# dmlc/xgboost

Hardware: AMD Instinct MI355X
Metric: boosting_rounds_per_sec (higher is better)
Workload: dtype fp32; 1 GPU; model=higgs-1m-hist, rows_per_gpu=1000000, n_features=28, max_depth=8, max_bin=256, objective=binary:logistic, parallelism=dp1, device=cuda

## Files before the change

### xgboost_amd/backend/gpu.py

```python
from __future__ import annotations

from typing import List, Optional, Sequence, Tuple

import numpy as np
import torch

from .. import collective
from ..data import QuantizedMatrix
from ..params import TrainParam
from ..splits import SplitEntry
from .cpu import GradQuantizer

LDS_MAX_GROUP_BINS = 8192
TARGET_HIST_TASKS = 2048
MIN_ROWS_PER_TASK = 1024


def _chunk_tasks(segments: Sequence[Tuple[int, int]],
                 slots: Optional[Sequence[int]] = None,
                 target_tasks: int = TARGET_HIST_TASKS,
                 min_rows: int = MIN_ROWS_PER_TASK) -> np.ndarray:
    total = sum(e - s for s, e in segments)
    rows_per_task = max(min_rows,
                        (total + target_tasks - 1) // max(target_tasks, 1))
# ... 507 lines not shown
                "pos": torch.zeros(n_rows, dtype=torch.int32, device=dev),
                "counters": torch.empty(max(4, 1 << param.max_depth),
                                        dtype=torch.int32, device=dev),
                "hist_tasks_cap": 16384 + max_build + 8,
                "hist_tasks": torch.empty((16384 + max_build + 8, 4),
                                          dtype=torch.int32, device=dev),
                "tg_scratch": torch.empty(3 * max_build + 8,
                                          dtype=torch.int32, device=dev),
                "qg_stage": torch.empty((n_rows, 2), dtype=torch.int32,
                                        device=dev),
                "rs_stage": torch.empty(2, dtype=torch.int64, device=dev),
                "ma_stage": torch.empty(2, dtype=torch.float32,
                                        device=dev),
                "fm_stage": torch.empty(self.qm.n_features,
                                        dtype=torch.uint8, device=dev),
                "driver": self.lib.gbt_driver_create(),
            }
            pool = 2 * max_build
            if pool <= 2048:
                rec = 1 + param.max_depth * pool
                mp = n_rows // 1024 + pool + 2
                wt_bytes = (48 * rec + 8 * rec + 8 * (param.max_depth + 2)
                            + 96 * pool + 32 * pool + 16 * mp
                            + param.max_depth * pool + 32 * 1024)
                ws["wt_max_ptasks"] = mp
                ws["wt_ws"] = torch.empty(wt_bytes, dtype=torch.uint8,
                                          device=dev)
            else:
                ws["wt_max_ptasks"] = 0
                ws["wt_ws"] = None
            self._native_ws = ws
        cap = 1 << (param.max_depth + 1)
        host = {name: np.zeros(cap, dt) for name, dt in [
            ("left", np.int32), ("right", np.int32), ("parent", np.int32),
            ("split_index", np.int32), ("split_cond", np.float32),
            ("default_left", np.uint8), ("loss_chg", np.float64),
            ("sum_hess", np.float32), ("base_weight", np.float32)]}
        fmask_ptr = None
        if feature_mask is not None:
            fm = np.ascontiguousarray(feature_mask, np.uint8)
            ws["fm_stage"].copy_(
                torch.from_numpy(fm), non_blocking=True)
            fmask_ptr = self.hip.ptr(ws["fm_stage"])
        mono_dev = mono_host = None
        if monotone is not None:
            m8 = np.ascontiguousarray(monotone, np.int8)
            key = m8.tobytes()
# ... 568 lines not shown
```

### xgboost_amd/ops/__init__.py

```python
from __future__ import annotations

import ctypes
import os
from typing import Optional

import torch

_HERE = os.path.dirname(os.path.abspath(__file__))
_LIB_PATH = os.path.join(_HERE, "libgbt_hip.so")
_lib: Optional[ctypes.CDLL] = None

_c = ctypes
_p = _c.c_void_p
_i = _c.c_int
_i64 = _c.c_int64
_f = _c.c_float
_d = _c.c_double

_SIGS = {
    "gbt_hist": [_p, _p, _i, _p, _p, _p, _i, _p, _i, _p, _p, _i, _i, _p, _i, _p, _p],
    "gbt_partition": [_p, _p, _i, _p, _p, _i64, _p, _p, _p, _i, _p, _p, _p,
                      _p, _p, _p, _p, _p],
    "gbt_evaluate": [_p, _i, _i, _i, _p, _p, _p, _d, _d, _d, _d, _d, _d,
                     _p, _p, _p, _p, _p, _p, _p, _p, _p, _i, _p],
# ... 1 lines not shown
    "gbt_predict": [_p, _i64, _i, _f, _i, _p, _p, _p, _p, _p, _p, _p, _p,
                    _p, _p, _i, _i, _p, _p, _p],
    "gbt_predict_q": [_p, _i, _i64, _i, _f, _i, _p, _p, _p, _p, _p, _p, _p,
                      _p, _i, _i, _p, _p, _p],
    "gbt_leaf_partition": [_p, _p, _i, _p, _p, _p],
    "gbt_leaf_decide": [_p, _p, _i, _p, _p, _i64, _p, _p, _i, _p, _p, _p,
                        _p, _p, _p, _p],
    "gbt_copy_ranges": [_p, _p, _p, _i, _p],
    "gbt_select_best": [_p, _p, _p, _p, _i, _i, _p, _p, _p],
    "gbt_mt_evaluate": [_p, _i, _i, _i, _i, _p, _p, _p, _p,
                        _d, _d, _d, _d, _p, _p, _p, _p, _p],
    "gbt_gpair_fused": [_i, _p, _p, _p, _f, _i64, _p, _p, _p],
    "gbt_quantize": [_p, _i64, _d, _d, _p, _p, _p, _p],
    "gbt_margin_add": [_p, _p, _p, _i64, _i, _i, _p],
    "gbt_hist_cpu": [_p, _p, _i, _p, _p, _p, _p, _i, _p, _p, _i],
    "gbt_partition_cpu": [_p, _p, _i, _p, _i64, _i64, _i, _i, _i, _p, _i,
                          _i, _p],
    "gbt_evaluate_cpu": [_p, _i, _i, _i, _p, _p, _d, _d, _d, _d, _d, _d,
                         _p, _p, _p, _p],
    "gbt_hist_csr": [_p, _p, _p, _p, _p, _i, _p, _i, _p],
    "gbt_partition_csr": [_p, _p, _p, _p, _p, _i, _p, _p, _p, _p, _p, _p],
    "gbt_driver_create": [],
    "gbt_driver_destroy": [_p],
    "gbt_grow_tree": [
        _p,
        _p, _p, _i,
        _p, _p,
        _i64, _p,
        _p, _p, _p, _p,
        _p, _p, _i, _i, _i, _i,
        _p, _p, _p, _p,
        _p, _p, _p, _p, _p, _p,
        _i,
        _p, _p, _i, _p,
        _p, _i64, _i,
        _p,
        _p, _p,
        _d, _d,
        _d, _d, _d, _d, _d, _d,
        _i,
        _p, _p,
        _p,
        _p,
        _p, _p, _p, _p, _p, _p, _p, _p, _p,
        _p,
    ],
# ... 14 lines not shown
    global _lib
    if _lib is not None:
        return _lib
    if not os.path.exists(_LIB_PATH):
        try:
            from .build_ext import build
            build()
        except Exception as e:
            raise RuntimeError(
                f"HIP kernel library missing and build failed: {e}. "
                f"Run `python {os.path.join(_HERE, 'build_ext.py')}`."
            ) from e
    _lib = ctypes.CDLL(_LIB_PATH)
    for name, argtypes in _SIGS.items():
        try:
            fn = getattr(_lib, name)
        except AttributeError:
            continue
        fn.argtypes = argtypes
        fn.restype = None
    if hasattr(_lib, "gbt_driver_create"):
        _lib.gbt_driver_create.restype = _p
        _lib.gbt_grow_tree.restype = _c.c_int
    if hasattr(_lib, "gbt_partition_cpu"):
        _lib.gbt_partition_cpu.restype = _c.c_longlong
    return _lib


ALLREDUCE_FN = _c.CFUNCTYPE(None, _c.POINTER(_c.c_longlong), _c.c_longlong)


def available() -> bool:
    try:
        load()
        return True
    except RuntimeError:
        return False


def ptr(t: Optional[torch.Tensor]):
    if t is None:
        return None
    assert t.is_contiguous(), "kernel arg tensors must be contiguous"
    return _c.c_void_p(t.data_ptr())


# ... 3 lines not shown
```

### xgboost_amd/ops/cpp/driver.hip

```cpp
#include "gbt_kernels.h"

#include <hip/hip_runtime.h>

#include <algorithm>
#include <cmath>
#include <cstdio>
#include <cstdlib>
#include <cstring>
#include <vector>

namespace {

#define HIP_CHECK(x)                                    \
  do {                                                  \
    hipError_t err__ = (x);                             \
    if (err__ != hipSuccess) return -(int)err__;        \
  } while (0)

struct PinnedRing {
  static constexpr int kSlots = 6;
  void* host[kSlots] = {};
  void* dev[kSlots] = {};
  size_t cap[kSlots] = {};
  int cur = 0;
// ... 4 lines not shown
    while (want < bytes) want <<= 1;
    if (host[slot]) hipHostFree(host[slot]);
    if (dev[slot]) hipFree(dev[slot]);
    HIP_CHECK(hipHostMalloc(&host[slot], want));
    HIP_CHECK(hipMalloc(&dev[slot], want));
    cap[slot] = want;
    return 0;
  }
  int next() {
    int s = cur;
    cur = (cur + 1) % kSlots;
    return s;
  }
};

struct DriverCtx {
  PinnedRing ring;
  void* readback_host = nullptr;
  size_t readback_cap = 0;

  hipGraphExec_t wt_graph = nullptr;
  std::vector<unsigned long long> wt_key;
  std::vector<unsigned long long> wt_seen_key;
  void* wtc_host = nullptr;
  void* wtc_dev = nullptr;
  size_t wtc_cap = 0;
  hipStream_t gstream = nullptr;
  hipEvent_t gevent = nullptr;

  int ensure_gstream() {
    if (gstream == nullptr)
      HIP_CHECK(hipStreamCreateWithFlags(&gstream, hipStreamNonBlocking));
    if (gevent == nullptr)
      HIP_CHECK(hipEventCreateWithFlags(&gevent, hipEventDisableTiming));
    return 0;
  }

  int ensure_readback(size_t bytes) {
    if (readback_cap >= bytes) return 0;
    size_t want = 4096;
    while (want < bytes) want <<= 1;
    if (readback_host) hipHostFree(readback_host);
    HIP_CHECK(hipHostMalloc(&readback_host, want));
    readback_cap = want;
    return 0;
  }
  int ensure_const(size_t bytes) {
    if (wtc_cap >= bytes) return 0;
    size_t want = 4096;
    while (want < bytes) want <<= 1;
    if (wtc_host) hipHostFree(wtc_host);
    if (wtc_dev) hipFree(wtc_dev);
    HIP_CHECK(hipHostMalloc(&wtc_host, want));
    HIP_CHECK(hipMalloc(&wtc_dev, want));
    wtc_cap = want;
    return 0;
  }
  ~DriverCtx() {
    for (int i = 0; i < PinnedRing::kSlots; ++i) {
      if (ring.host[i]) hipHostFree(ring.host[i]);
      if (ring.dev[i]) hipFree(ring.dev[i]);
    }
    if (readback_host) hipHostFree(readback_host);
    if (wt_graph) (void)hipGraphExecDestroy(wt_graph);
    if (wtc_host) hipHostFree(wtc_host);
    if (wtc_dev) hipFree(wtc_dev);
    if (gstream) (void)hipStreamDestroy(gstream);
    if (gevent) (void)hipEventDestroy(gevent);
  }
};

bool WtGraphEnabled() {
  static int v = [] {
    const char* e = getenv("GBT_WT_GRAPH");
    return e ? atoi(e) : 1;
  }();
  return v != 0;
}

bool WtGraphDebug() {
  static int v = [] {
    const char* e = getenv("GBT_WT_GRAPH_DEBUG");
    return e ? atoi(e) : 0;
  }();
  return v != 0;
}

struct Node {
  int nid;
// ... 45 lines not shown
  for (auto* n : nodes) total += n->seg_end - n->seg_begin;
  long long rows_per_task =
      std::max<long long>(min_rows, (total + target_tasks - 1) / target_tasks);
  for (size_t i = 0; i < nodes.size(); ++i) {
    int b = nodes[i]->seg_begin;
    while (b < nodes[i]->seg_end) {
      int e = (int)std::min<long long>(b + rows_per_task, nodes[i]->seg_end);
      out->push_back(BlockTask{(int)i, b, e, 0});
      b = e;
    }
  }
  if (out->empty()) out->push_back(BlockTask{0, 0, 0, 0});
}

__global__ void ZeroI64Kernel(int64_t* p, long long n) {
  long long i = (long long)blockIdx.x * blockDim.x + threadIdx.x;
  long long stride = (long long)gridDim.x * blockDim.x;
  for (; i < n; i += stride) p[i] = 0;
}

__global__ void IotaKernel(int32_t* r, long long n) {
  long long i = (long long)blockIdx.x * blockDim.x + threadIdx.x;
  for (; i < n; i += (long long)gridDim.x * blockDim.x) r[i] = (int)i;
}

__global__ void SubtractHistKernel(const int64_t* __restrict__ parents,
                                   const int64_t* __restrict__ built,
                                   int64_t* __restrict__ out,
                                   const int32_t* __restrict__ parent_slot,
                                   int n_bins2, int k,
                                   int64_t* __restrict__ ps,
                                   const int64_t* __restrict__ parent_ps,
                                   const int32_t* __restrict__ kp_dev) {
  if (kp_dev != nullptr) {
    k = *kp_dev;
    out += (long long)k * n_bins2;
  }
  const long long idx = (long long)blockIdx.x * blockDim.x + threadIdx.x;
  if (ps != nullptr && idx < k) {
    ps[2 * (k + idx)] = parent_ps[2 * idx] - ps[2 * idx];
    ps[2 * (k + idx) + 1] = parent_ps[2 * idx + 1] - ps[2 * idx + 1];
  }
  const long long total = (long long)k * n_bins2;
  for (long long i = idx; i < total; i += (long long)gridDim.x * blockDim.x) {
    const int row = (int)(i / n_bins2);
    const int col = (int)(i % n_bins2);
// ... 247 lines not shown
      const int mid = (lo + hi + 1) >> 1;
      if (s_pref[mid] <= t) lo = mid; else hi = mid - 1;
    }
    const int j = lo;
    const long long idx = t - s_pref[j];
    const int b = s_b[j] + (int)(idx * rpt);
    const int e = (int)std::min<long long>((long long)b + rpt,
                                           (long long)s_e[j]);
    out_tasks[t] = BlockTask{j, b, e, 0};
  }
}

struct LeafSeg {
  int nid, begin, end;
  int parity;
};

}

extern "C" {

void* gbt_driver_create() { return new DriverCtx(); }
void gbt_driver_destroy(void* ctx) { delete (DriverCtx*)ctx; }

typedef void (*AllreduceFn)(long long* dev_ptr, long long n_elems);

int gbt_grow_tree(
    void* vctx, const uint8_t* gidx8, const uint16_t* gidx16, int n_features,
    const uint8_t* gidx8_col, const uint16_t* gidx16_col,
    long long n_rows, const int32_t* qgpair, const int32_t* cut_ptrs_dev,
    const float* cut_values_host, const int32_t* cut_ptrs_host,
    const int32_t* n_bins_feat_dev, const int32_t* feat_group_start_dev,
    const int32_t* bin_group_start_dev, int n_groups, int max_group_bins,
    int use_shared, int n_bins,
    int32_t* ridx, int32_t* ridx_out, int64_t* hist_pool_a,
    int64_t* hist_pool_b, double* eval_gain, int32_t* eval_bin,
    uint8_t* eval_dir, int64_t* eval_lsum, int64_t* eval_best,
    int32_t* pos_out, int max_nodes_level,
    int32_t* part_counters,
    BlockTask* hist_tasks_dev,
    int hist_tasks_cap,
    int32_t* tg_scratch,
    void* wt_ws,
    long long wt_ws_bytes, int wt_max_ptasks,
    const int64_t* root_sums_dev,
    const float* maxabs_dev,
// ... 28 lines not shown
  }
  int32_t* cur_ridx = ridx;
  int32_t* alt_ridx = ridx_out;

  int n_tree_nodes = 1;
  out_left[0] = -1;
  out_right[0] = -1;
  out_parent[0] = -1;

  Node root{};
  root.nid = 0;
  root.seg_begin = 0;
  root.seg_end = (int)n_rows;
  root.hist_slot = 0;
  root.lo = -INFINITY;
  root.hi = INFINITY;

  static long long hist_tasks = [] {
    const char* e = getenv("GBT_HIST_TASKS");
    long long v = e ? atoll(e) : 256;
    return v >= 64 && v <= 16384 ? v : 256;
  }();
  const long long hist_min_rows = 2048;

  if (!whole_tree) {
    std::vector<Node*> nodes{&root};
    std::vector<BlockTask> tasks;
    ChunkTasks(nodes, &tasks, hist_min_rows, hist_tasks);
    const int slot = ctx->ring.next();
    size_t bytes = tasks.size() * sizeof(BlockTask);
    if (int e = ctx->ring.ensure(slot, bytes)) return e;
    memcpy(ctx->ring.host[slot], tasks.data(), bytes);
    HIP_CHECK(hipMemcpyAsync(ctx->ring.dev[slot], ctx->ring.host[slot], bytes,
                             hipMemcpyHostToDevice, stream));
    HIP_CHECK(hipMemsetAsync(hist_pool_a, 0, hist_row * sizeof(int64_t),
                             stream));
    gbt_hist(gidx8, gidx16, n_features, qgpair, ridx,
             (const BlockTask*)ctx->ring.dev[slot], (int)tasks.size(),
             hist_pool_a, n_bins, feat_group_start_dev, bin_group_start_dev,
             n_groups, max_group_bins, cut_ptrs_dev, use_shared, nullptr,
             stream);
    if (allreduce) allreduce((long long*)hist_pool_a, hist_row);
  }

  auto evaluate_enqueue = [&](int k, std::vector<Node*>* nodes,
                              const int64_t* hists, const int64_t* ps_dev,
// ... 81 lines not shown
    *best_out = (const int64_t*)(h + off_best);
    *cnt_out = (const int32_t*)(h + off_cnt);
    return 0;
  };

  std::vector<Node> level_nodes;
  std::vector<Node> next_level;
  std::vector<LeafSeg> leaves;
  int64_t* cur_pool = hist_pool_a;
  int64_t* next_pool = hist_pool_b;

  if (whole_tree) {
    const int choice_global = (allreduce != nullptr || has_mono) ? 1 : 0;
    const int pool = 2 * max_nodes_level;
    const int rec_slots = 1 + max_depth * pool;
    size_t off = 0;
    auto carve = [&](size_t bytes) {
      size_t o = off;
      off = (off + bytes + 255) & ~255ULL;
      return o;
    };
    const size_t o_best = carve((size_t)rec_slots * 6 * 8);
    const size_t o_seg = carve((size_t)rec_slots * 2 * 4);
    const size_t o_kn = carve((size_t)(max_depth + 2) * 4);
    const size_t o_kp = carve((size_t)(max_depth + 2) * 4);
    const size_t o_descw = carve((size_t)pool * 16);
    const size_t o_featw = carve((size_t)pool * 4);
    const size_t o_sbinw = carve((size_t)pool * 4);
    const size_t o_dlw = carve((size_t)pool);
    const size_t o_cntw = carve((size_t)pool * 8);
    const size_t o_pt = carve((size_t)wt_max_ptasks * sizeof(BlockTask));
    const size_t o_pps = carve((size_t)pool * 16);
    const size_t o_pslot = carve((size_t)pool * 4);
    const size_t o_psa = carve((size_t)pool * 16);
    const size_t o_psb = carve((size_t)pool * 16);
    const size_t o_bnda = has_mono ? carve((size_t)pool * 16) : 0;
    const size_t o_bndb = has_mono ? carve((size_t)pool * 16) : 0;
    const size_t o_mode = carve((size_t)max_depth * pool);
    if ((long long)off > wt_ws_bytes) return -9997;
    char* w = (char*)wt_ws;
    int64_t* best_rec = (int64_t*)(w + o_best);
    int32_t* seg_rec = (int32_t*)(w + o_seg);
    int32_t* kn_arr = (int32_t*)(w + o_kn);
    int32_t* kp_arr = (int32_t*)(w + o_kp);
    int32_t* d_desc = (int32_t*)(w + o_descw);
    int32_t* d_feat = (int32_t*)(w + o_featw);
    int32_t* d_sbin = (int32_t*)(w + o_sbinw);
    uint8_t* d_dl = (uint8_t*)(w + o_dlw);
    int32_t* d_cnt = (int32_t*)(w + o_cntw);
    BlockTask* d_pt = (BlockTask*)(w + o_pt);
    int64_t* d_pps = (int64_t*)(w + o_pps);
    int32_t* d_pslot = (int32_t*)(w + o_pslot);
    int64_t* ps_bufs[2] = {(int64_t*)(w + o_psa), (int64_t*)(w + o_psb)};
    double* bnd_bufs[2] = {
        has_mono ? (double*)(w + o_bnda) : nullptr,
        has_mono ? (double*)(w + o_bndb) : nullptr};
    uint8_t* d_mode = (uint8_t*)(w + o_mode);

    std::vector<BlockTask> rtasks;
    {
      std::vector<Node*> rnodes{&root};
      ChunkTasks(rnodes, &rtasks, hist_min_rows, hist_tasks);
    }
    const size_t c_tasks_off = 16;
    if (int e = ctx->ensure_const(c_tasks_off +
                                  rtasks.size() * sizeof(BlockTask)))
      return e;
    {
      int32_t* hh = (int32_t*)ctx->wtc_host;
      hh[0] = 1;
      hh[1] = 0;
      hh[2] = 0;
      hh[3] = (int)n_rows;
      memcpy((char*)ctx->wtc_host + c_tasks_off, rtasks.data(),
             rtasks.size() * sizeof(BlockTask));
    }
    const int wt_max_htasks = (int)std::min<long long>(
        std::min<long long>(n_rows / hist_min_rows, hist_tasks) +
            max_nodes_level + 1,
        (long long)hist_tasks_cap);
    size_t r_best = 0;
    size_t r_seg = ((size_t)rec_slots * 48 + 63) & ~63ULL;
    size_t r_kp = (r_seg + (size_t)rec_slots * 8 + 63) & ~63ULL;
    size_t r_rs = (r_kp + (size_t)(max_depth + 2) * 4 + 63) & ~63ULL;
    size_t r_ma = r_rs + 16;
    size_t r_mode = (r_ma + 8 + 63) & ~63ULL;
    size_t r_total = r_mode + (size_t)max_depth * pool;
    if (int e = ctx->ensure_readback(r_total)) return e;
    char* rb = (char*)ctx->readback_host;

    auto stage_h2d = [&](hipStream_t cs) -> int {
      char* ch = (char*)ctx->wtc_host;
      HIP_CHECK(hipMemcpyAsync(kn_arr, ch, 4, hipMemcpyHostToDevice,
                               cs));
      HIP_CHECK(hipMemcpyAsync(kp_arr, ch + 4, 4, hipMemcpyHostToDevice,
                               cs));
      HIP_CHECK(hipMemcpyAsync(seg_rec, ch + 8, 8, hipMemcpyHostToDevice,
                               cs));
      HIP_CHECK(hipMemcpyAsync((char*)ctx->wtc_dev + c_tasks_off,
                               ch + c_tasks_off,
                               rtasks.size() * sizeof(BlockTask),
                               hipMemcpyHostToDevice, cs));
      return 0;
    };
    auto enqueue_chain = [&](hipStream_t cs) -> int {
      int32_t* cr = ridx;
      int32_t* ar = ridx_out;
      int64_t* cp = hist_pool_a;
      int64_t* np2 = hist_pool_b;
      {
        int blocks = (int)std::min<long long>((n_rows + 255) / 256, 4096);
        hipLaunchKernelGGL(IotaKernel, dim3(blocks), dim3(256), 0, cs,
                           cr, n_rows);
      }
      {
        int zb = (int)std::min<long long>((hist_row + 255) / 256, 4096);
        hipLaunchKernelGGL(ZeroI64Kernel, dim3(zb), dim3(256), 0, cs, cp,
                           hist_row);
      }
      gbt_hist(gidx8, gidx16, n_features, qgpair, cr,
               (const BlockTask*)((char*)ctx->wtc_dev + c_tasks_off),
               (int)rtasks.size(), cp, n_bins, feat_group_start_dev,
               bin_group_start_dev, n_groups, max_group_bins, cut_ptrs_dev,
               use_shared, nullptr, cs);
      if (allreduce) allreduce((long long*)cp, hist_row);
      gbt_evaluate_masked(cp, 1, n_bins, n_features, cut_ptrs_dev,
                   root_sums_dev, maxabs_dev, 0.0, 0.0, reg_lambda,
                   reg_alpha, max_delta_step, min_child_weight,
                   has_mono ? monotone_dev : nullptr, nullptr,
                   0 , fmask_dev,
                   nullptr, eval_gain, eval_bin, eval_dir, eval_lsum,
                   nullptr, 0, cs);
      gbt_select_best(eval_gain, eval_bin, eval_dir, eval_lsum, 1,
                      n_features, best_rec, nullptr, cs);
      const int64_t* ps_prev = root_sums_dev;
      for (int L = 0; L + 1 < max_depth; ++L) {
        const int64_t* bl =
            best_rec + (L == 0 ? 0 : (1 + (size_t)(L - 1) * pool) * 6);
        const int32_t* sl =
            seg_rec + (L == 0 ? 0 : (1 + (size_t)(L - 1) * pool) * 2);
        int64_t* bo = best_rec + (1 + (size_t)L * pool) * 6;
        int32_t* so = seg_rec + (1 + (size_t)L * pool) * 2;
        int64_t* ps_next = ps_bufs[L & 1];
        const int cap_kids =
            (int)std::min<long long>(2LL << L, (long long)pool);
        hipLaunchKernelGGL(ApplyKernel, dim3(1), dim3(256), 0, cs, bl,
                           sl, kn_arr + L, kp_arr + L, ps_prev, gamma,
                           cut_ptrs_dev,
                           (long long)1024, (long long)2048, wt_max_ptasks,
                           kn_arr + L + 1, kp_arr + L + 1, d_feat, d_sbin,
                           d_dl, d_cnt, d_pt, d_desc, d_pps, d_pslot,
                           choice_global, maxabs_dev,
                           has_mono ? monotone_dev : nullptr,
                           reg_lambda, reg_alpha, max_delta_step,
                           (L == 0 || !has_mono) ? nullptr
                                                 : bnd_bufs[(L - 1) & 1],
                           has_mono ? bnd_bufs[L & 1] : nullptr,
                           L == 0 ? nullptr : d_mode + (size_t)(L - 1) * pool);
        gbt_partition(gidx8, gidx16, n_features, gidx8_col, gidx16_col,
                      n_rows, cr, ar, d_pt,
                      wt_max_ptasks, d_feat, d_sbin, d_dl, nullptr, nullptr,
                      n_bins_feat_dev, d_cnt, cs);
        std::swap(cr, ar);
        hipLaunchKernelGGL(HistTaskGenKernel, dim3(1), dim3(256), 0, cs,
                           d_cnt, d_desc, 0, hist_min_rows, hist_tasks,
                           wt_max_htasks, tg_scratch, hist_tasks_dev,
                           ps_next, kp_arr + L + 1, so,
                           allreduce != nullptr ? 2 * cap_kids : 0,
                           d_mode + (size_t)L * pool);
        {
          const long long zn = (long long)cap_kids * hist_row;
          int zb = (int)std::min<long long>((zn + 255) / 256, 4096);
          hipLaunchKernelGGL(ZeroI64Kernel, dim3(zb), dim3(256), 0, cs,
                             np2, zn);
        }
        gbt_hist(gidx8, gidx16, n_features, qgpair, cr, hist_tasks_dev,
                 wt_max_htasks, np2, n_bins, feat_group_start_dev,
                 bin_group_start_dev, n_groups, max_group_bins,
                 cut_ptrs_dev, use_shared, ps_next, cs);
        if (allreduce) {
          allreduce((long long*)np2,
                    (long long)(cap_kids / 2) * hist_row);
          allreduce((long long*)ps_next, (long long)cap_kids);
        }
// ... 1 lines not shown
          const long long total = (long long)(cap_kids / 2 + 1) * hist_row;
          int blocks = (int)std::min<long long>((total + 255) / 256, 4096);
          hipLaunchKernelGGL(SubtractHistKernel, dim3(blocks), dim3(256), 0,
                             cs, cp, np2, np2, d_pslot,
                             (int)hist_row, 0, ps_next, d_pps,
                             kp_arr + L + 1);
        }
        gbt_evaluate_masked(np2, cap_kids, n_bins, n_features, cut_ptrs_dev,
                     ps_next, maxabs_dev, 0.0, 0.0, reg_lambda, reg_alpha,
                     max_delta_step, min_child_weight,
                     has_mono ? monotone_dev : nullptr,
                     has_mono ? bnd_bufs[L & 1] : nullptr,
                     0 , fmask_dev, nullptr, eval_gain,
                     eval_bin, eval_dir, eval_lsum, kn_arr + L + 1, 0,
                     cs);
        gbt_select_best(eval_gain, eval_bin, eval_dir, eval_lsum, cap_kids,
                        n_features, bo, kn_arr + L + 1, cs);
        ps_prev = ps_next;
        std::swap(cp, np2);
      }
      return 0;
    };
    auto readback = [&](hipStream_t cs) -> int {
      HIP_CHECK(hipMemcpyAsync(rb + r_best, best_rec,
                               (size_t)rec_slots * 48,
                               hipMemcpyDeviceToHost, cs));
      HIP_CHECK(hipMemcpyAsync(rb + r_seg, seg_rec, (size_t)rec_slots * 8,
                               hipMemcpyDeviceToHost, cs));
      HIP_CHECK(hipMemcpyAsync(rb + r_kp, kp_arr,
                               (size_t)(max_depth + 2) * 4,
                               hipMemcpyDeviceToHost, cs));
      HIP_CHECK(hipMemcpyAsync(rb + r_rs, root_sums_dev, 16,
                               hipMemcpyDeviceToHost, cs));
      HIP_CHECK(hipMemcpyAsync(rb + r_ma, maxabs_dev, 8,
                               hipMemcpyDeviceToHost, cs));
      HIP_CHECK(hipMemcpyAsync(rb + r_mode, d_mode,
                               (size_t)max_depth * pool,
                               hipMemcpyDeviceToHost, cs));
      return 0;
    };

    bool enqueued = false;
    if (allreduce == nullptr && WtGraphEnabled() &&
        ctx->ensure_gstream() == 0) {
      auto db = [](double d) {
        unsigned long long u;
        memcpy(&u, &d, 8);
        return u;
      };
      std::vector<unsigned long long> key = {
          (unsigned long long)gidx8, (unsigned long long)gidx16,
          (unsigned long long)gidx8_col, (unsigned long long)gidx16_col,
          (unsigned long long)qgpair, (unsigned long long)cut_ptrs_dev,
          (unsigned long long)n_bins_feat_dev,
          (unsigned long long)feat_group_start_dev,
          (unsigned long long)bin_group_start_dev,
          (unsigned long long)ridx, (unsigned long long)ridx_out,
          (unsigned long long)hist_pool_a, (unsigned long long)hist_pool_b,
          (unsigned long long)eval_gain, (unsigned long long)eval_bin,
          (unsigned long long)eval_dir, (unsigned long long)eval_lsum,
          (unsigned long long)hist_tasks_dev,
          (unsigned long long)tg_scratch, (unsigned long long)wt_ws,
          (unsigned long long)root_sums_dev,
          (unsigned long long)maxabs_dev, (unsigned long long)monotone_dev,
          (unsigned long long)fmask_dev,
          (unsigned long long)ctx->readback_host,
          (unsigned long long)ctx->wtc_host,
          (unsigned long long)ctx->wtc_dev,
          (unsigned long long)n_rows, (unsigned long long)n_features,
          (unsigned long long)n_bins, (unsigned long long)use_shared,
          (unsigned long long)n_groups,
          (unsigned long long)max_group_bins,
          (unsigned long long)max_depth,
          (unsigned long long)max_nodes_level,
          (unsigned long long)wt_max_ptasks,
          (unsigned long long)hist_tasks_cap,
          (unsigned long long)rtasks.size(),
          (unsigned long long)has_mono,
          db(reg_lambda), db(reg_alpha), db(max_delta_step),
          db(min_child_weight), db(gamma)};
      HIP_CHECK(hipEventRecord(ctx->gevent, stream));
      HIP_CHECK(hipEventSynchronize(ctx->gevent));
      if (ctx->wt_graph != nullptr && key == ctx->wt_key) {
        if (int e = stage_h2d(ctx->gstream)) return e;
        if (hipGraphLaunch(ctx->wt_graph, ctx->gstream) == hipSuccess) {
          enqueued = true;
          if (WtGraphDebug()) fprintf(stderr, "[wtgraph] replay\n");
        } else {
          (void)hipGetLastError();
          (void)hipGraphExecDestroy(ctx->wt_graph);
          ctx->wt_graph = nullptr;
          ctx->wt_key.clear();
        }
      }
      if (!enqueued && key != ctx->wt_seen_key) {
        ctx->wt_seen_key = key;
      } else if (!enqueued) {
        if (int e = stage_h2d(ctx->gstream)) return e;
        if (hipStreamBeginCapture(ctx->gstream,
                                  hipStreamCaptureModeRelaxed) !=
            hipSuccess) {
          (void)hipGetLastError();
          goto graph_done;
        }
        int ec = enqueue_chain(ctx->gstream);
        hipGraph_t g = nullptr;
        hipError_t ce = hipStreamEndCapture(ctx->gstream, &g);
        if (WtGraphDebug())
          fprintf(stderr, "[wtgraph] capture ec=%d end=%d\n", ec, (int)ce);
        if (ec != 0) {
          if (g) (void)hipGraphDestroy(g);
          return ec;
        }
        if (ce == hipSuccess && g != nullptr) {
          if (ctx->wt_graph) {
            (void)hipGraphExecDestroy(ctx->wt_graph);
            ctx->wt_graph = nullptr;
          }
          ctx->wt_key.clear();
          hipError_t ie =
              hipGraphInstantiate(&ctx->wt_graph, g, nullptr, nullptr, 0);
// ... 8 lines not shown
            enqueued = true;
          } else if (ctx->wt_graph) {
            (void)hipGraphExecDestroy(ctx->wt_graph);
            ctx->wt_graph = nullptr;
          }
          (void)hipGraphDestroy(g);
        } else {
          (void)hipGetLastError();
        }
      }
    graph_done:
      if (!enqueued) {
        hipStreamCaptureStatus st = hipStreamCaptureStatusNone;
        if (hipStreamIsCapturing(ctx->gstream, &st) == hipSuccess &&
            st != hipStreamCaptureStatusNone) {
          hipGraph_t junk = nullptr;
          (void)hipStreamEndCapture(ctx->gstream, &junk);
          if (junk) (void)hipGraphDestroy(junk);
        }
      }
    }
    if (!enqueued) {
      if (WtGraphDebug()) fprintf(stderr, "[wtgraph] direct enqueue\n");
      if (int e = stage_h2d(stream)) return e;
      if (int e = enqueue_chain(stream)) return e;
      if (int e = readback(stream)) return e;
    } else {
      if (int e = readback(ctx->gstream)) return e;
      HIP_CHECK(hipStreamSynchronize(ctx->gstream));
    }
    HIP_CHECK(hipStreamSynchronize(stream));
    if ((max_depth - 1) & 1) std::swap(cur_ridx, alt_ridx);
    const int64_t* h_best = (const int64_t*)(rb + r_best);
    const int32_t* h_seg = (const int32_t*)(rb + r_seg);
    const int32_t* h_kp = (const int32_t*)(rb + r_kp);
    const int64_t* h_rs = (const int64_t*)(rb + r_rs);
    const float* h_ma = (const float*)(rb + r_ma);
    const uint8_t* h_mode = (const uint8_t*)(rb + r_mode);
    g_scale = h_ma[0] > 0.f ? 1073741824.0 / (double)h_ma[0] : 1.0;
    h_scale = h_ma[1] > 0.f ? 1073741824.0 / (double)h_ma[1] : 1.0;
    inv_g = 1.0 / g_scale;
    inv_h = 1.0 / h_scale;
    if (out_scales != nullptr) {
      out_scales[0] = g_scale;
      out_scales[1] = h_scale;
    }
    root.gq = h_rs[0];
    root.hq = h_rs[1];
    out_base_weight[0] =
        (float)CalcWeight(root.gq * inv_g, root.hq * inv_h, p);
    out_sum_hess[0] = (float)(root.hq * inv_h);
    {
      double gn;
      memcpy(&gn, &h_best[0], 8);
      root.bin = (int)h_best[1];
      root.dir = (int)h_best[2];
      root.lgq = h_best[3];
      root.lhq = h_best[4];
      root.feature = (int)h_best[5];
      root.gain = (root.bin >= 0 && std::isfinite(gn)) ? gn : -INFINITY;
    }
// ... 485 lines not shown
```

### xgboost_amd/ops/cpp/partition.hip

```cpp
#include "gbt_kernels.h"

#ifndef GBT_PART_BLOCK
#define GBT_PART_BLOCK 256
#endif

__device__ __forceinline__ bool DecideLeft(int local_bin, int fbins,
                                           int split_bin_local,
                                           bool default_left,
                                           const uint32_t* cat_bits,
                                           int cat_words) {
  if (local_bin >= fbins) {
    return default_left;
  }
  if (cat_words > 0) {
    const int w = local_bin >> 5;
    const bool in_set =
        (w < cat_words) && ((cat_bits[w] >> (local_bin & 31)) & 1u);
    return !in_set;
  }
  return local_bin <= split_bin_local;
}

template <typename BinT>
__global__ __launch_bounds__(GBT_PART_BLOCK) void PartitionKernel(
    const BinT* __restrict__ gidx, int n_features,
    const BinT* __restrict__ gidx_col, long long col_ld,
    const int32_t* __restrict__ ridx_in, int32_t* __restrict__ ridx_out,
    const BlockTask* __restrict__ tasks,
    const int32_t* __restrict__ split_feature,
    const int32_t* __restrict__ split_bin_local,
    const uint8_t* __restrict__ default_left,
    const uint32_t* __restrict__ cat_bits,
    const int32_t* __restrict__ cat_bits_offset,
    const int32_t* __restrict__ n_bins_feat,
    int32_t* __restrict__ counters) {
  const BlockTask task = tasks[blockIdx.x];
  if (task.row_begin >= task.row_end) return;
  const int slot = task.out_slot;
  const int feature = split_feature[slot];
  const int sbin = split_bin_local[slot];
  const bool dleft = default_left[slot] != 0;
  const int fbins = n_bins_feat[feature];
  const uint32_t* cats = nullptr;
  int cat_words = 0;
  if (cat_bits_offset != nullptr) {
    const int c0 = cat_bits_offset[slot];
    cat_words = cat_bits_offset[slot + 1] - c0;
    if (cat_words > 0) cats = cat_bits + c0;
  }

  const int n_rows = task.row_end - task.row_begin;
  const int chunk = (n_rows + (int)blockDim.x - 1) / (int)blockDim.x;
  const int my_begin = task.row_begin + (int)threadIdx.x * chunk;
  const int my_end = min(my_begin + chunk, task.row_end);

  constexpr int kMaxCacheRows = 65536;
  __shared__ uint32_t decide_bits[kMaxCacheRows / 32];
  const bool use_cache = n_rows <= kMaxCacheRows;
  if (use_cache) {
    const int n_words = (n_rows + 31) / 32;
    for (int i = threadIdx.x; i < n_words; i += blockDim.x) {
      decide_bits[i] = 0u;
    }
    __syncthreads();
  }

  const BinT* col = gidx_col ? gidx_col + (size_t)feature * col_ld
                             : nullptr;
  int my_left = 0;
  for (int i = my_begin; i < my_end; ++i) {
    const int row = ridx_in[i];
    const int local = col ? (int)col[row]
                          : (int)gidx[(size_t)row * n_features + feature];
    const bool left = DecideLeft(local, fbins, sbin, dleft, cats, cat_words);
    my_left += left ? 1 : 0;
    if (use_cache) {
      const int k = i - task.row_begin;
      if (left) atomicOr(&decide_bits[k >> 5], 1u << (k & 31));
    }
  }
  const int my_rows = max(my_end - my_begin, 0);
  const int my_right = my_rows - my_left;

  __shared__ int wave_left[GBT_PART_BLOCK / 64];
  __shared__ int wave_right[GBT_PART_BLOCK / 64];
  __shared__ int base_l, base_r;
  const int lane = threadIdx.x & 63;
  const int wave = threadIdx.x >> 6;
  int scan_l = my_left, scan_r = my_right;
  for (int off = 1; off < 64; off <<= 1) {
    const int tl = __shfl_up(scan_l, off, 64);
    const int tr = __shfl_up(scan_r, off, 64);
    if (lane >= off) {
      scan_l += tl;
      scan_r += tr;
    }
  }
  if (lane == 63) {
    wave_left[wave] = scan_l;
    wave_right[wave] = scan_r;
  }
  __syncthreads();
  int wl_off = 0, wr_off = 0;
  for (int w = 0; w < wave; ++w) {
    wl_off += wave_left[w];
    wr_off += wave_right[w];
  }
  const int excl_l = scan_l - my_left + wl_off;
  const int excl_r = scan_r - my_right + wr_off;
  if (threadIdx.x == (int)blockDim.x - 1) {
    const int tot_l = excl_l + my_left;
    const int tot_r = excl_r + my_right;
    base_l = tot_l ? atomicAdd(&counters[2 * slot], tot_l) : 0;
    base_r = tot_r ? atomicSub(&counters[2 * slot + 1], tot_r) - tot_r : 0;
  }
  __syncthreads();

  int dl = base_l + excl_l;
  int dr = base_r + excl_r;
  for (int i = my_begin; i < my_end; ++i) {
    const int row = ridx_in[i];
    bool left;
    if (use_cache) {
      const int k = i - task.row_begin;
      left = (decide_bits[k >> 5] >> (k & 31)) & 1u;
    } else {
      const int local = col ? (int)col[row]
                            : (int)gidx[(size_t)row * n_features + feature];
      left = DecideLeft(local, fbins, sbin, dleft, cats, cat_words);
    }
    if (left) {
      ridx_out[dl++] = row;
    } else {
      ridx_out[dr++] = row;
    }
  }
}

extern "C" void gbt_partition(
    const uint8_t* gidx8, const uint16_t* gidx16, int n_features,
    const uint8_t* gidx8_col, const uint16_t* gidx16_col, int64_t col_ld,
    const int32_t* ridx_in, int32_t* ridx_out, const BlockTask* tasks,
    int n_tasks, const int32_t* split_feature, const int32_t* split_bin_local,
    const uint8_t* default_left, const uint32_t* cat_bits,
    const int32_t* cat_bits_offset, const int32_t* n_bins_feat,
    int32_t* counters, hipStream_t stream) {
  if (gidx8 != nullptr) {
    hipLaunchKernelGGL((PartitionKernel<uint8_t>), dim3(n_tasks),
                       dim3(GBT_PART_BLOCK), 0, stream, gidx8, n_features,
                       gidx8_col, (long long)col_ld,
                       ridx_in, ridx_out, tasks, split_feature,
                       split_bin_local, default_left, cat_bits,
                       cat_bits_offset, n_bins_feat, counters);
  } else {
    hipLaunchKernelGGL((PartitionKernel<uint16_t>), dim3(n_tasks),
                       dim3(GBT_PART_BLOCK), 0, stream, gidx16, n_features,
                       gidx16_col, (long long)col_ld,
                       ridx_in, ridx_out, tasks, split_feature,
// ... 98 lines not shown
```

Baseline: 931.9 rounds/s.

## Rewrite partition kernel with wave ballots and fuse whole-tree init on device

The partition kernel now has each wave classify 64 consecutive rows with ballot and mbcnt, keeping decisions in registers instead of per-thread strided chunks with LDS atomicOr bit caches. Writes become coalesced within a wave, and there are separate tile-count variants by task size. Host-side root task staging and H2D copies are replaced by a fused device init kernel that also does iota and zeroing, and the readback is packed into one contiguous memcpy. Partition task granularity becomes tunable (default 4096 rows, launching fewer partition tasks). A debug check function for root tasks is also added.

```diff
diff --git a/xgboost_amd/backend/gpu.py b/xgboost_amd/backend/gpu.py
--- a/xgboost_amd/backend/gpu.py
+++ b/xgboost_amd/backend/gpu.py
@@ -553,7 +553,7 @@
                 mp = n_rows // 1024 + pool + 2
                 wt_bytes = (48 * rec + 8 * rec + 8 * (param.max_depth + 2)
                             + 96 * pool + 32 * pool + 16 * mp
-                            + param.max_depth * pool + 32 * 1024)
+                            + param.max_depth * pool + 24 + 32 * 1024)
                 ws["wt_max_ptasks"] = mp
                 ws["wt_ws"] = torch.empty(wt_bytes, dtype=torch.uint8,
                                           device=dev)
diff --git a/xgboost_amd/ops/__init__.py b/xgboost_amd/ops/__init__.py
--- a/xgboost_amd/ops/__init__.py
+++ b/xgboost_amd/ops/__init__.py
@@ -47,6 +47,7 @@
     "gbt_partition_csr": [_p, _p, _p, _p, _p, _i, _p, _p, _p, _p, _p, _p],
     "gbt_driver_create": [],
     "gbt_driver_destroy": [_p],
+    "gbt_root_tasks_check": [_i64, _i64, _i64, _p],
     "gbt_grow_tree": [
         _p,
         _p, _p, _i,
@@ -107,6 +108,8 @@
     if hasattr(_lib, "gbt_driver_create"):
         _lib.gbt_driver_create.restype = _p
         _lib.gbt_grow_tree.restype = _c.c_int
+    if hasattr(_lib, "gbt_root_tasks_check"):
+        _lib.gbt_root_tasks_check.restype = _c.c_int
     if hasattr(_lib, "gbt_partition_cpu"):
         _lib.gbt_partition_cpu.restype = _c.c_longlong
     return _lib
diff --git a/xgboost_amd/ops/cpp/driver.hip b/xgboost_amd/ops/cpp/driver.hip
--- a/xgboost_amd/ops/cpp/driver.hip
+++ b/xgboost_amd/ops/cpp/driver.hip
@@ -50,9 +50,6 @@
   hipGraphExec_t wt_graph = nullptr;
   std::vector<unsigned long long> wt_key;
   std::vector<unsigned long long> wt_seen_key;
-  void* wtc_host = nullptr;
-  void* wtc_dev = nullptr;
-  size_t wtc_cap = 0;
   hipStream_t gstream = nullptr;
   hipEvent_t gevent = nullptr;
 
@@ -73,17 +70,6 @@
     readback_cap = want;
     return 0;
   }
-  int ensure_const(size_t bytes) {
-    if (wtc_cap >= bytes) return 0;
-    size_t want = 4096;
-    while (want < bytes) want <<= 1;
-    if (wtc_host) hipHostFree(wtc_host);
-    if (wtc_dev) hipFree(wtc_dev);
-    HIP_CHECK(hipHostMalloc(&wtc_host, want));
-    HIP_CHECK(hipMalloc(&wtc_dev, want));
-    wtc_cap = want;
-    return 0;
-  }
   ~DriverCtx() {
     for (int i = 0; i < PinnedRing::kSlots; ++i) {
       if (ring.host[i]) hipHostFree(ring.host[i]);
@@ -91,8 +77,6 @@
     }
     if (readback_host) hipHostFree(readback_host);
     if (wt_graph) (void)hipGraphExecDestroy(wt_graph);
-    if (wtc_host) hipHostFree(wtc_host);
-    if (wtc_dev) hipFree(wtc_dev);
     if (gstream) (void)hipStreamDestroy(gstream);
     if (gevent) (void)hipEventDestroy(gevent);
   }
@@ -184,6 +168,45 @@
 __global__ void IotaKernel(int32_t* r, long long n) {
   long long i = (long long)blockIdx.x * blockDim.x + threadIdx.x;
   for (; i < n; i += (long long)gridDim.x * blockDim.x) r[i] = (int)i;
+}
+
+long long RootRowsPerTask(long long n_rows, long long min_rows,
+                          long long target_tasks) {
+  return std::max<long long>(min_rows,
+                             (n_rows + target_tasks - 1) / target_tasks);
+}
+int RootTaskCount(long long n_rows, long long rpt) {
+  return (int)std::max<long long>(1, (n_rows + rpt - 1) / rpt);
+}
+
+__global__ void WtInitKernel(int32_t* r, long long n, int64_t* zero,
+                             long long zero_n, int32_t* kn, int32_t* kp,
+                             int32_t* seg, BlockTask* root_tasks,
+                             int n_root_tasks, long long rpt,
+                             const int64_t* __restrict__ root_sums,
+                             const float* __restrict__ maxabs,
+                             int64_t* rs_out ) {
+  const long long stride = (long long)gridDim.x * blockDim.x;
+  const long long i0 = (long long)blockIdx.x * blockDim.x + threadIdx.x;
+  for (long long i = i0; i < n; i += stride) r[i] = (int)i;
+  for (long long i = i0; i < zero_n; i += stride) zero[i] = 0;
+  if (blockIdx.x != 0) return;
+  if (threadIdx.x == 0) {
+    kn[0] = 1;
+    kp[0] = 0;
+    seg[0] = 0;
+    seg[1] = (int)n;
+    rs_out[0] = root_sums[0];
+    rs_out[1] = root_sums[1];
+    float* ma = (float*)(rs_out + 2);
+    ma[0] = maxabs[0];
+    ma[1] = maxabs[1];
+  }
+  for (int t = threadIdx.x; t < n_root_tasks; t += blockDim.x) {
+    const long long b = (long long)t * rpt;
+    root_tasks[t] =
+        BlockTask{0, (int)b, (int)std::min<long long>(b + rpt, n), 0};
+  }
 }
 
 __global__ void SubtractHistKernel(const int64_t* __restrict__ parents,
@@ -477,6 +500,48 @@
 
 void* gbt_driver_create() { return new DriverCtx(); }
 void gbt_driver_destroy(void* ctx) { delete (DriverCtx*)ctx; }
+
+int gbt_root_tasks_check(long long n_rows, long long min_rows,
+                         long long target_tasks, void* stream_v) {
+  hipStream_t stream = (hipStream_t)stream_v;
+  Node root{};
+  root.seg_end = (int)n_rows;
+  std::vector<Node*> nodes{&root};
+  std::vector<BlockTask> want;
+  ChunkTasks(nodes, &want, min_rows, target_tasks);
+  const long long rpt = RootRowsPerTask(n_rows, min_rows, target_tasks);
+  const int nt = RootTaskCount(n_rows, rpt);
+  const size_t o_tasks = 192;
+  const size_t o_ridx = o_tasks + (size_t)nt * sizeof(BlockTask);
+  const size_t bytes = o_ridx + (size_t)std::max<long long>(n_rows, 1) * 4;
+  char* d = nullptr;
+  HIP_CHECK(hipMalloc((void**)&d, bytes));
+  int rc = 0;
+  std::vector<BlockTask> got(nt);
+  hipError_t e = hipMemsetAsync(d, 0, o_tasks, stream);
+  if (e == hipSuccess) {
+    int32_t* sc = (int32_t*)d;
+    hipLaunchKernelGGL(WtInitKernel, dim3(2), dim3(256), 0, stream,
+                       (int32_t*)(d + o_ridx), n_rows, (int64_t*)nullptr,
+                       0LL, sc, sc + 1, sc + 2, (BlockTask*)(d + o_tasks),
+                       nt, rpt, (const int64_t*)(d + 64),
+                       (const float*)(d + 80), (int64_t*)(d + 128));
+    e = hipMemcpyAsync(got.data(), d + o_tasks,
+                       (size_t)nt * sizeof(BlockTask), hipMemcpyDeviceToHost,
+                       stream);
+  }
+  if (e == hipSuccess) e = hipStreamSynchronize(stream);
+  (void)hipFree(d);
+  if (e != hipSuccess) return -(int)e;
+  if (want.size() != got.size()) return (int)std::max(want.size(), got.size());
+  for (size_t i = 0; i < want.size(); ++i) {
+    if (want[i].out_slot != got[i].out_slot ||
+        want[i].row_begin != got[i].row_begin ||
+        want[i].row_end != got[i].row_end)
+      ++rc;
+  }
+  return rc;
+}
 
 typedef void (*AllreduceFn)(long long* dev_ptr, long long n_elems);
 
@@ -551,6 +616,11 @@
     return v >= 64 && v <= 16384 ? v : 256;
   }();
   const long long hist_min_rows = 2048;
+  static long long part_min_rows = [] {
+    const char* e = getenv("GBT_PART_ROWS");
+    long long v = e ? atoll(e) : 4096;
+    return v >= 1024 && v <= 65536 && (v & (v - 1)) == 0 ? v : 4096;
+  }();
 
   if (!whole_tree) {
     std::vector<Node*> nodes{&root};
@@ -678,8 +748,11 @@
     };
     const size_t o_best = carve((size_t)rec_slots * 6 * 8);
     const size_t o_seg = carve((size_t)rec_slots * 2 * 4);
+    const size_t o_kp = carve((size_t)(max_depth + 2) * 4);
+    const size_t o_mode = carve((size_t)max_depth * pool);
+    const size_t o_rs = carve(24);
+    const size_t r_total = o_rs + 24;
     const size_t o_kn = carve((size_t)(max_depth + 2) * 4);
-    const size_t o_kp = carve((size_t)(max_depth + 2) * 4);
     const size_t o_descw = carve((size_t)pool * 16);
     const size_t o_featw = carve((size_t)pool * 4);
     const size_t o_sbinw = carve((size_t)pool * 4);
@@ -692,7 +765,6 @@
     const size_t o_psb = carve((size_t)pool * 16);
     const size_t o_bnda = has_mono ? carve((size_t)pool * 16) : 0;
     const size_t o_bndb = has_mono ? carve((size_t)pool * 16) : 0;
-    const size_t o_mode = carve((size_t)max_depth * pool);
     if ((long long)off > wt_ws_bytes) return -9997;
     char* w = (char*)wt_ws;
     int64_t* best_rec = (int64_t*)(w + o_best);
@@ -713,52 +785,20 @@
         has_mono ? (double*)(w + o_bndb) : nullptr};
     uint8_t* d_mode = (uint8_t*)(w + o_mode);
 
-    std::vector<BlockTask> rtasks;
-    {
-      std::vector<Node*> rnodes{&root};
-      ChunkTasks(rnodes, &rtasks, hist_min_rows, hist_tasks);
-    }
-    const size_t c_tasks_off = 16;
-    if (int e = ctx->ensure_const(c_tasks_off +
-                                  rtasks.size() * sizeof(BlockTask)))
-      return e;
-    {
-      int32_t* hh = (int32_t*)ctx->wtc_host;
-      hh[0] = 1;
-      hh[1] = 0;
-      hh[2] = 0;
-      hh[3] = (int)n_rows;
-      memcpy((char*)ctx->wtc_host + c_tasks_off, rtasks.data(),
-             rtasks.size() * sizeof(BlockTask));
-    }
+    const long long root_rpt =
+        RootRowsPerTask(n_rows, hist_min_rows, hist_tasks);
+    const int n_root_tasks = RootTaskCount(n_rows, root_rpt);
+    if (n_root_tasks > hist_tasks_cap) return -9996;
+    int64_t* d_rs = (int64_t*)(w + o_rs);
     const int wt_max_htasks = (int)std::min<long long>(
         std::min<long long>(n_rows / hist_min_rows, hist_tasks) +
             max_nodes_level + 1,
         (long long)hist_tasks_cap);
-    size_t r_best = 0;
-    size_t r_seg = ((size_t)rec_slots * 48 + 63) & ~63ULL;
-    size_t r_kp = (r_seg + (size_t)rec_slots * 8 + 63) & ~63ULL;
-    size_t r_rs = (r_kp + (size_t)(max_depth + 2) * 4 + 63) & ~63ULL;
-    size_t r_ma = r_rs + 16;
-    size_t r_mode = (r_ma + 8 + 63) & ~63ULL;
-    size_t r_total = r_mode + (size_t)max_depth * pool;
+    const int n_ptasks = (int)std::min<long long>(
+        n_rows / part_min_rows + pool + 2, (long long)wt_max_ptasks);
     if (int e = ctx->ensure_readback(r_total)) return e;
     char* rb = (char*)ctx->readback_host;
 
-    auto stage_h2d = [&](hipStream_t cs) -> int {
-      char* ch = (char*)ctx->wtc_host;
-      HIP_CHECK(hipMemcpyAsync(kn_arr, ch, 4, hipMemcpyHostToDevice,
-                               cs));
-      HIP_CHECK(hipMemcpyAsync(kp_arr, ch + 4, 4, hipMemcpyHostToDevice,
-                               cs));
-      HIP_CHECK(hipMemcpyAsync(seg_rec, ch + 8, 8, hipMemcpyHostToDevice,
-                               cs));
-      HIP_CHECK(hipMemcpyAsync((char*)ctx->wtc_dev + c_tasks_off,
-                               ch + c_tasks_off,
-                               rtasks.size() * sizeof(BlockTask),
-                               hipMemcpyHostToDevice, cs));
-      return 0;
-    };
     auto enqueue_chain = [&](hipStream_t cs) -> int {
       int32_t* cr = ridx;
       int32_t* ar = ridx_out;
@@ -766,17 +806,15 @@
       int64_t* np2 = hist_pool_b;
       {
         int blocks = (int)std::min<long long>((n_rows + 255) / 256, 4096);
-        hipLaunchKernelGGL(IotaKernel, dim3(blocks), dim3(256), 0, cs,
-                           cr, n_rows);
-      }
-      {
-        int zb = (int)std::min<long long>((hist_row + 255) / 256, 4096);
-        hipLaunchKernelGGL(ZeroI64Kernel, dim3(zb), dim3(256), 0, cs, cp,
-                           hist_row);
+        hipLaunchKernelGGL(WtInitKernel, dim3(std::max(blocks, 1)),
+                           dim3(256), 0, cs, cr, n_rows, cp, hist_row,
+                           kn_arr, kp_arr, seg_rec, hist_tasks_dev,
+                           n_root_tasks, root_rpt, root_sums_dev, maxabs_dev,
+                           d_rs);
       }
       gbt_hist(gidx8, gidx16, n_features, qgpair, cr,
-               (const BlockTask*)((char*)ctx->wtc_dev + c_tasks_off),
-               (int)rtasks.size(), cp, n_bins, feat_group_start_dev,
+               hist_tasks_dev, n_root_tasks, cp, n_bins,
+               feat_group_start_dev,
                bin_group_start_dev, n_groups, max_group_bins, cut_ptrs_dev,
                use_shared, nullptr, cs);
       if (allreduce) allreduce((long long*)cp, hist_row);
@@ -803,7 +841,7 @@
         hipLaunchKernelGGL(ApplyKernel, dim3(1), dim3(256), 0, cs, bl,
                            sl, kn_arr + L, kp_arr + L, ps_prev, gamma,
                            cut_ptrs_dev,
-                           (long long)1024, (long long)2048, wt_max_ptasks,
+                           part_min_rows, (long long)2048, n_ptasks,
                            kn_arr + L + 1, kp_arr + L + 1, d_feat, d_sbin,
                            d_dl, d_cnt, d_pt, d_desc, d_pps, d_pslot,
                            choice_global, maxabs_dev,
@@ -815,7 +853,7 @@
                            L == 0 ? nullptr : d_mode + (size_t)(L - 1) * pool);
         gbt_partition(gidx8, gidx16, n_features, gidx8_col, gidx16_col,
                       n_rows, cr, ar, d_pt,
-                      wt_max_ptasks, d_feat, d_sbin, d_dl, nullptr, nullptr,
+                      n_ptasks, d_feat, d_sbin, d_dl, nullptr, nullptr,
                       n_bins_feat_dev, d_cnt, cs);
         std::swap(cr, ar);
         hipLaunchKernelGGL(HistTaskGenKernel, dim3(1), dim3(256), 0, cs,
@@ -863,20 +901,7 @@
       return 0;
     };
     auto readback = [&](hipStream_t cs) -> int {
-      HIP_CHECK(hipMemcpyAsync(rb + r_best, best_rec,
-                               (size_t)rec_slots * 48,
-                               hipMemcpyDeviceToHost, cs));
-      HIP_CHECK(hipMemcpyAsync(rb + r_seg, seg_rec, (size_t)rec_slots * 8,
-                               hipMemcpyDeviceToHost, cs));
-      HIP_CHECK(hipMemcpyAsync(rb + r_kp, kp_arr,
-                               (size_t)(max_depth + 2) * 4,
-                               hipMemcpyDeviceToHost, cs));
-      HIP_CHECK(hipMemcpyAsync(rb + r_rs, root_sums_dev, 16,
-                               hipMemcpyDeviceToHost, cs));
-      HIP_CHECK(hipMemcpyAsync(rb + r_ma, maxabs_dev, 8,
-                               hipMemcpyDeviceToHost, cs));
-      HIP_CHECK(hipMemcpyAsync(rb + r_mode, d_mode,
-                               (size_t)max_depth * pool,
+      HIP_CHECK(hipMemcpyAsync(rb, w + o_best, r_total,
                                hipMemcpyDeviceToHost, cs));
       return 0;
     };
@@ -906,8 +931,6 @@
           (unsigned long long)maxabs_dev, (unsigned long long)monotone_dev,
           (unsigned long long)fmask_dev,
           (unsigned long long)ctx->readback_host,
-          (unsigned long long)ctx->wtc_host,
-          (unsigned long long)ctx->wtc_dev,
           (unsigned long long)n_rows, (unsigned long long)n_features,
           (unsigned long long)n_bins, (unsigned long long)use_shared,
           (unsigned long long)n_groups,
@@ -916,14 +939,17 @@
           (unsigned long long)max_nodes_level,
           (unsigned long long)wt_max_ptasks,
           (unsigned long long)hist_tasks_cap,
-          (unsigned long long)rtasks.size(),
+          (unsigned long long)n_root_tasks,
+          (unsigned long long)root_rpt,
+          (unsigned long long)part_min_rows,
+          (unsigned long long)n_ptasks,
+          (unsigned long long)wt_max_htasks,
           (unsigned long long)has_mono,
           db(reg_lambda), db(reg_alpha), db(max_delta_step),
           db(min_child_weight), db(gamma)};
       HIP_CHECK(hipEventRecord(ctx->gevent, stream));
       HIP_CHECK(hipEventSynchronize(ctx->gevent));
       if (ctx->wt_graph != nullptr && key == ctx->wt_key) {
-        if (int e = stage_h2d(ctx->gstream)) return e;
         if (hipGraphLaunch(ctx->wt_graph, ctx->gstream) == hipSuccess) {
           enqueued = true;
           if (WtGraphDebug()) fprintf(stderr, "[wtgraph] replay\n");
@@ -937,7 +963,6 @@
       if (!enqueued && key != ctx->wt_seen_key) {
         ctx->wt_seen_key = key;
       } else if (!enqueued) {
-        if (int e = stage_h2d(ctx->gstream)) return e;
         if (hipStreamBeginCapture(ctx->gstream,
                                   hipStreamCaptureModeRelaxed) !=
             hipSuccess) {
@@ -992,7 +1017,6 @@
     }
     if (!enqueued) {
       if (WtGraphDebug()) fprintf(stderr, "[wtgraph] direct enqueue\n");
-      if (int e = stage_h2d(stream)) return e;
       if (int e = enqueue_chain(stream)) return e;
       if (int e = readback(stream)) return e;
     } else {
@@ -1001,12 +1025,12 @@
     }
     HIP_CHECK(hipStreamSynchronize(stream));
     if ((max_depth - 1) & 1) std::swap(cur_ridx, alt_ridx);
-    const int64_t* h_best = (const int64_t*)(rb + r_best);
-    const int32_t* h_seg = (const int32_t*)(rb + r_seg);
-    const int32_t* h_kp = (const int32_t*)(rb + r_kp);
-    const int64_t* h_rs = (const int64_t*)(rb + r_rs);
-    const float* h_ma = (const float*)(rb + r_ma);
-    const uint8_t* h_mode = (const uint8_t*)(rb + r_mode);
+    const int64_t* h_best = (const int64_t*)(rb + o_best);
+    const int32_t* h_seg = (const int32_t*)(rb + o_seg);
+    const int32_t* h_kp = (const int32_t*)(rb + o_kp);
+    const int64_t* h_rs = (const int64_t*)(rb + o_rs);
+    const float* h_ma = (const float*)(rb + o_rs + 16);
+    const uint8_t* h_mode = (const uint8_t*)(rb + o_mode);
     g_scale = h_ma[0] > 0.f ? 1073741824.0 / (double)h_ma[0] : 1.0;
     h_scale = h_ma[1] > 0.f ? 1073741824.0 / (double)h_ma[1] : 1.0;
     inv_g = 1.0 / g_scale;
diff --git a/xgboost_amd/ops/cpp/partition.hip b/xgboost_amd/ops/cpp/partition.hip
--- a/xgboost_amd/ops/cpp/partition.hip
+++ b/xgboost_amd/ops/cpp/partition.hip
@@ -3,6 +3,13 @@
 #ifndef GBT_PART_BLOCK
 #define GBT_PART_BLOCK 256
 #endif
+
+namespace {
+constexpr int kPartWaves = GBT_PART_BLOCK / 64;
+constexpr int kPartTilesSmall = 4;
+constexpr int kPartTilesLarge = 16;
+constexpr int kPartCacheRows = kPartTilesLarge * 64 * kPartWaves;
+}
 
 __device__ __forceinline__ bool DecideLeft(int local_bin, int fbins,
                                            int split_bin_local,
@@ -19,6 +26,132 @@
     return !in_set;
   }
   return local_bin <= split_bin_local;
+}
+
+template <typename BinT>
+struct PartSplit {
+  const BinT* gidx;
+  const BinT* col;
+  int n_features, feature, fbins, sbin, cat_words;
+  bool dleft;
+  const uint32_t* cats;
+
+  __device__ __forceinline__ bool Left(int row) const {
+    const int local = col ? (int)col[row]
+                          : (int)gidx[(size_t)row * n_features + feature];
+    return DecideLeft(local, fbins, sbin, dleft, cats, cat_words);
+  }
+};
+
+__device__ __forceinline__ int LanesBelow(unsigned long long m) {
+  return (int)__builtin_amdgcn_mbcnt_hi(
+      (unsigned)(m >> 32), __builtin_amdgcn_mbcnt_lo((unsigned)m, 0u));
+}
+
+__device__ __forceinline__ void ReserveWindows(int wave_left, int wave_right,
+                                               int32_t* counters, int slot,
+                                               int* dl, int* dr) {
+  __shared__ int s_left[kPartWaves], s_right[kPartWaves];
+  __shared__ int s_base_l, s_base_r;
+  const int lane = threadIdx.x & 63;
+  const int wave = threadIdx.x >> 6;
+  if (lane == 0) {
+    s_left[wave] = wave_left;
+    s_right[wave] = wave_right;
+  }
+  __syncthreads();
+  if (threadIdx.x == 0) {
+    int tot_l = 0, tot_r = 0;
+    for (int w = 0; w < kPartWaves; ++w) {
+      tot_l += s_left[w];
+      tot_r += s_right[w];
+    }
+    s_base_l = tot_l ? atomicAdd(&counters[2 * slot], tot_l) : 0;
+    s_base_r = tot_r ? atomicSub(&counters[2 * slot + 1], tot_r) - tot_r : 0;
+  }
+  __syncthreads();
+  int l = s_base_l, r = s_base_r;
+  for (int w = 0; w < wave; ++w) {
+    l += s_left[w];
+    r += s_right[w];
+  }
+  *dl = l;
+  *dr = r;
+}
+
+template <typename BinT, int TILES>
+__device__ __forceinline__ void PartitionCached(
+    const PartSplit<BinT>& sp, const int32_t* __restrict__ ridx_in,
+    int32_t* __restrict__ ridx_out, int begin, int end, int slot,
+    int32_t* counters) {
+  const int lane = threadIdx.x & 63;
+  const int wave = threadIdx.x >> 6;
+  int rows[TILES];
+  unsigned long long lmask[TILES];
+  int wave_left = 0, wave_rows = 0;
+#pragma unroll
+  for (int j = 0; j < TILES; ++j) {
+    const int i = begin + (j * kPartWaves + wave) * 64 + lane;
+    const bool valid = i < end;
+    rows[j] = ridx_in[min(i, end - 1)];
+    lmask[j] = __ballot(sp.Left(rows[j]) && valid);
+    wave_left += __popcll(lmask[j]);
+    wave_rows += __popcll(__ballot(valid));
+  }
+  int dl, dr;
+  ReserveWindows(wave_left, wave_rows - wave_left, counters, slot, &dl, &dr);
+#pragma unroll
+  for (int j = 0; j < TILES; ++j) {
+    const int i = begin + (j * kPartWaves + wave) * 64 + lane;
+    const bool valid = i < end;
+    const unsigned long long lm = lmask[j];
+    const unsigned long long rm = __ballot(valid) & ~lm;
+    if (valid) {
+      if ((lm >> lane) & 1ull) {
+        ridx_out[dl + LanesBelow(lm)] = rows[j];
+      } else {
+        ridx_out[dr + LanesBelow(rm)] = rows[j];
+      }
+    }
+    dl += __popcll(lm);
+    dr += __popcll(rm);
+  }
+}
+
+template <typename BinT>
+__device__ __forceinline__ void PartitionRegather(
+    const PartSplit<BinT>& sp, const int32_t* __restrict__ ridx_in,
+    int32_t* __restrict__ ridx_out, int begin, int end, int slot,
+    int32_t* counters) {
+  const int lane = threadIdx.x & 63;
+  const int wave = threadIdx.x >> 6;
+  int wave_left = 0, wave_rows = 0;
+  for (int t0 = begin + wave * 64; t0 < end; t0 += kPartWaves * 64) {
+    const int i = t0 + lane;
+    const bool valid = i < end;
+    const int row = ridx_in[min(i, end - 1)];
+    wave_left += __popcll(__ballot(sp.Left(row) && valid));
+    wave_rows += __popcll(__ballot(valid));
+  }
+  int dl, dr;
+  ReserveWindows(wave_left, wave_rows - wave_left, counters, slot, &dl, &dr);
+  for (int t0 = begin + wave * 64; t0 < end; t0 += kPartWaves * 64) {
+    const int i = t0 + lane;
+    const bool valid = i < end;
+    const int row = ridx_in[min(i, end - 1)];
+    const bool left = sp.Left(row) && valid;
+    const unsigned long long lm = __ballot(left);
+    const unsigned long long rm = __ballot(valid) & ~lm;
+    if (valid) {
+      if (left) {
+        ridx_out[dl + LanesBelow(lm)] = row;
+      } else {
+        ridx_out[dr + LanesBelow(rm)] = row;
+      }
+    }
+    dl += __popcll(lm);
+    dr += __popcll(rm);
+  }
 }
 
 template <typename BinT>
@@ -37,103 +170,34 @@
   const BlockTask task = tasks[blockIdx.x];
   if (task.row_begin >= task.row_end) return;
   const int slot = task.out_slot;
-  const int feature = split_feature[slot];
-  const int sbin = split_bin_local[slot];
-  const bool dleft = default_left[slot] != 0;
-  const int fbins = n_bins_feat[feature];
-  const uint32_t* cats = nullptr;
-  int cat_words = 0;
+  PartSplit<BinT> sp;
+  sp.gidx = gidx;
+  sp.n_features = n_features;
+  sp.feature = split_feature[slot];
+  sp.sbin = split_bin_local[slot];
+  sp.dleft = default_left[slot] != 0;
+  sp.fbins = n_bins_feat[sp.feature];
+  sp.cats = nullptr;
+  sp.cat_words = 0;
   if (cat_bits_offset != nullptr) {
     const int c0 = cat_bits_offset[slot];
-    cat_words = cat_bits_offset[slot + 1] - c0;
-    if (cat_words > 0) cats = cat_bits + c0;
-  }
+    sp.cat_words = cat_bits_offset[slot + 1] - c0;
+    if (sp.cat_words > 0) sp.cats = cat_bits + c0;
+  }
+  sp.col = gidx_col ? gidx_col + (size_t)sp.feature * col_ld : nullptr;
 
   const int n_rows = task.row_end - task.row_begin;
-  const int chunk = (n_rows + (int)blockDim.x - 1) / (int)blockDim.x;
-  const int my_begin = task.row_begin + (int)threadIdx.x * chunk;
-  const int my_end = min(my_begin + chunk, task.row_end);
-
-  constexpr int kMaxCacheRows = 65536;
-  __shared__ uint32_t decide_bits[kMaxCacheRows / 32];
-  const bool use_cache = n_rows <= kMaxCacheRows;
-  if (use_cache) {
-    const int n_words = (n_rows + 31) / 32;
-    for (int i = threadIdx.x; i < n_words; i += blockDim.x) {
-      decide_bits[i] = 0u;
-    }
-    __syncthreads();
-  }
-
-  const BinT* col = gidx_col ? gidx_col + (size_t)feature * col_ld
-                             : nullptr;
-  int my_left = 0;
-  for (int i = my_begin; i < my_end; ++i) {
-    const int row = ridx_in[i];
-    const int local = col ? (int)col[row]
-                          : (int)gidx[(size_t)row * n_features + feature];
-    const bool left = DecideLeft(local, fbins, sbin, dleft, cats, cat_words);
-    my_left += left ? 1 : 0;
-    if (use_cache) {
-      const int k = i - task.row_begin;
-      if (left) atomicOr(&decide_bits[k >> 5], 1u << (k & 31));
-    }
-  }
-  const int my_rows = max(my_end - my_begin, 0);
-  const int my_right = my_rows - my_left;
-
-  __shared__ int wave_left[GBT_PART_BLOCK / 64];
-  __shared__ int wave_right[GBT_PART_BLOCK / 64];
-  __shared__ int base_l, base_r;
-  const int lane = threadIdx.x & 63;
-  const int wave = threadIdx.x >> 6;
-  int scan_l = my_left, scan_r = my_right;
-  for (int off = 1; off < 64; off <<= 1) {
-    const int tl = __shfl_up(scan_l, off, 64);
-    const int tr = __shfl_up(scan_r, off, 64);
-    if (lane >= off) {
-      scan_l += tl;
-      scan_r += tr;
-    }
-  }
-  if (lane == 63) {
-    wave_left[wave] = scan_l;
-    wave_right[wave] = scan_r;
-  }
-  __syncthreads();
-  int wl_off = 0, wr_off = 0;
-  for (int w = 0; w < wave; ++w) {
-    wl_off += wave_left[w];
-    wr_off += wave_right[w];
-  }
-  const int excl_l = scan_l - my_left + wl_off;
-  const int excl_r = scan_r - my_right + wr_off;
-  if (threadIdx.x == (int)blockDim.x - 1) {
-    const int tot_l = excl_l + my_left;
-    const int tot_r = excl_r + my_right;
-    base_l = tot_l ? atomicAdd(&counters[2 * slot], tot_l) : 0;
-    base_r = tot_r ? atomicSub(&counters[2 * slot + 1], tot_r) - tot_r : 0;
-  }
-  __syncthreads();
-
-  int dl = base_l + excl_l;
-  int dr = base_r + excl_r;
-  for (int i = my_begin; i < my_end; ++i) {
-    const int row = ridx_in[i];
-    bool left;
-    if (use_cache) {
-      const int k = i - task.row_begin;
-      left = (decide_bits[k >> 5] >> (k & 31)) & 1u;
-    } else {
-      const int local = col ? (int)col[row]
-                            : (int)gidx[(size_t)row * n_features + feature];
-      left = DecideLeft(local, fbins, sbin, dleft, cats, cat_words);
-    }
-    if (left) {
-      ridx_out[dl++] = row;
-    } else {
-      ridx_out[dr++] = row;
-    }
+  if (n_rows <= kPartTilesSmall * 64 * kPartWaves) {
+    PartitionCached<BinT, kPartTilesSmall>(sp, ridx_in, ridx_out,
+                                           task.row_begin, task.row_end, slot,
+                                           counters);
+  } else if (n_rows <= kPartCacheRows) {
+    PartitionCached<BinT, kPartTilesLarge>(sp, ridx_in, ridx_out,
+                                           task.row_begin, task.row_end, slot,
+                                           counters);
+  } else {
+    PartitionRegather<BinT>(sp, ridx_in, ridx_out, task.row_begin,
+                            task.row_end, slot, counters);
   }
 }
 
```

Result: faster. 1021 rounds/s (median of 6 runs) (+9.6%).
